# jeanfeydy/geomloss

Measured on AMD Instinct MI355X. Metric: softmin pairs/s, N=M=1e6 3D fp32 (Sinkhorn wall-clock: `sinkhorn_wallclock`; roofline: `roofline`), higher is better.
Workload: dtype f32

## Files before the change

### geomloss_amd/csrc/glhip_api.hip

```cpp
#include "glhip_autosort.h"
#include "glhip_launch.h"

namespace glhip {
thread_local char g_err[512] = "";
}

#define GL_NBP(DD) XdShape<DD>::NBP
static const int kXdNBP[] = {GL_NBP(4), GL_NBP(5), GL_NBP(6), GL_NBP(7), GL_NBP(8), GL_NBP(9), GL_NBP(10), GL_NBP(11), GL_NBP(12), GL_NBP(13), GL_NBP(14), GL_NBP(15), GL_NBP(16)};
#undef GL_NBP
static_assert(sizeof kXdNBP / sizeof kXdNBP[0] == kXdMaxD - 3, "one entry per dimension of the xd kernels");

extern "C" {

int glhip_version(void) { return GLHIP_VERSION; }

size_t glhip_workspace_bytes(int B, int N, int M, int D, int n_ranges) {
    const int nr = X32Layout<XL_BF16X3>::NR, nbp = (D > 3 && D <= kXdMaxD) ? kXdNBP[D - 4] : 0;
    size_t bytes = forward_workspace_bytes(B, N, M, D, n_ranges, nr, nbp);
    if (bytes > 0 && autosort_applies(B, N, M, D, n_ranges, 0)) {
        const size_t sorted = autosort_bytes(N, M, D) + forward_workspace_bytes(1, N, M, D, (N + kSortSlab - 1) / kSortSlab, nr, nbp);
        bytes = bytes > sorted ? bytes : sorted;
    }
    return bytes;
}
// ... 12 lines not shown
        sc.l2.groups = static_cast<const GroupBox*>(a.groups);
        sc.l2.home = a.home;
        sc.l2.t2 = a.t2;
        sc.l2.centre_x = x;
        sc.l2.n_groups = (M + 31) / 32;
        sc.l2.L2 = (float)(prune_L(M) * 1.4426950408889634);
    }
    const Ranges rg{a.ranges_i, a.slices_i, a.red};
    return (in_dtype == GLHIP_F32) ? softmin_fwd_typed<float>(fn, a.xs, a.ys, h, a.out, 1, N, M, D, eps, p, rg, a.C, sc, inner, st, step)
                                   : softmin_fwd_typed<bf16_t>(fn, a.xs, a.ys, h, a.out, 1, N, M, D, eps, p, rg, a.C, sc, inner, st, step);
}

int glhip_softmin_fwd_family(int B, long N, long M, int D, int p, int dtype, int flags, int n_ranges) {
    if (B < 0 || N < 0 || M < 0 || N > 0x7fffffffL || M > 0x7fffffffL || D < 1 || n_ranges < 0 || (p != 1 && p != 2) ||
        (dtype != GLHIP_F32 && dtype != GLHIP_BF16))
        return GLHIP_EINVAL;
    if (softmin_sorts(B, (int)N, (int)M, D, p, n_ranges, flags))
        return softmin_fwd_family(1, N, M, D, p, flags | (p == 1 ? GLHIP_FLAG_MFMA_DIST : 0) | GLHIP_FLAG_NO_SORT, (int)((N + kSortSlab - 1) / kSortSlab));
    return softmin_fwd_family(B, N, M, D, p, flags, n_ranges);
}

int glhip_softmin_perm_applies(int B, long N, long M, int D, int p, int dtype, int flags, int n_ranges) {
    if (B < 0 || N < 0 || M < 0 || N > 0x7fffffffL || M > 0x7fffffffL || D < 1 || n_ranges < 0 || (p != 1 && p != 2) ||
        (dtype != GLHIP_F32 && dtype != GLHIP_BF16))
        return GLHIP_EINVAL;
    return p == 2 && softmin_sorts(B, (int)N, (int)M, D, p, n_ranges, flags) ? 1 : 0;
}

static int softmin_step(const char* fn, const void* x, const void* y, const float* logw, const float* pot, const float* prev, float* out, int B,
                        int N, int M, int D, float eps, float damping, int p, int in_dtype, const int32_t* ranges_i, const int32_t* slices_i,
                        const int32_t* redranges_j, int n_ranges, void* workspace, size_t workspace_bytes, int flags, void* stream,
                        int32_t* perm_x = nullptr, int32_t* perm_y = nullptr, int perm_flags = 0) {
    int rc = check_common(fn, x, y, logw, B, N, M, D, in_dtype, ranges_i, slices_i, redranges_j, n_ranges);
    if (rc) return rc;
    if (B == 0 || N == 0) return GLHIP_OK;
    if (!out) return fail(GLHIP_EINVAL, "%s: NULL out", fn);
    if (out == prev) return fail(GLHIP_EINVAL, "%s: out must not alias prev (updates are simultaneous)", fn);
    if (!(eps > 0.f)) return fail(GLHIP_EINVAL, "%s: eps must be > 0", fn);
    if (p != 1 && p != 2) return fail(GLHIP_EUNSUPPORTED, "%s: p must be 1 or 2 (got %d)", fn, p);
    hipStream_t st = static_cast<hipStream_t>(stream);
    StepArgs step{pot, prev, prev ? 0.5f * damping : damping, prev ? 0.5f : 0.f};
    if (softmin_sorts(B, N, M, D, p, n_ranges, flags)) {
        AutoSort a;
        const int C = (N + kSortSlab - 1) / kSortSlab;
        rc = autosort_prepare(a, x, y, N, M, D, in_dtype, workspace, workspace_bytes, glhip_workspace_bytes(1, N, M, D, C), st, p == 1, perm_x,
                              perm_y, perm_flags);
        if (rc) return rc;
        if (a.on) {
            gather_f32(logw, a.perm_y, a.col0, M, st, a.hint_y);
            if (pot) { gather_f32(pot, a.perm_y, a.col1, M, st, a.hint_y); step.pot = a.col1; }
            if (prev) { gather_f32(prev, a.perm_x, a.row0, N, st, a.hint_x); step.prev = a.row0; }
            if (p == 2)
                prune_ranges(a.xs, a.ys, a.col0, step.pot, 1.0f / eps, N, M, D, in_dtype, eps, a.ranges_i, a.slices_i, a.red, a.blocks, a.groups, a.home,
                             a.t2, a.mlb, a.t1, st);
            rc = sorted_inner(fn, a, x, a.col0, N, M, D, eps, p, in_dtype, flags, st, step);
            if (rc) return rc;
            scatter_f32(a.out, a.perm_x, out, N, st, 1, a.hint_x);
            return check_launch(fn);
        }
    }
    const Ranges rg{ranges_i, slices_i, redranges_j};
    const Scratch sc = make_scratch(workspace, workspace_bytes, flags, n_ranges, N);
    rc = (in_dtype == GLHIP_F32) ? softmin_fwd_typed<float>(fn, x, y, logw, out, B, N, M, D, eps, p, rg, n_ranges, sc, flags, st, step)
                                 : softmin_fwd_typed<bf16_t>(fn, x, y, logw, out, B, N, M, D, eps, p, rg, n_ranges, sc, flags, st, step);
    return rc ? rc : check_launch(fn);
}

int glhip_softmin_fwd(const void* x, const void* y, const float* h, float* out, int B, int N, int M, int D,
                      float eps, int p, int in_dtype, const int32_t* ranges_i, const int32_t* slices_i,
                      const int32_t* redranges_j, int n_ranges, void* workspace, size_t workspace_bytes, int flags,
                      void* stream) {
    return softmin_step("glhip_softmin_fwd", x, y, h, nullptr, nullptr, out, B, N, M, D, eps, 1.f, p, in_dtype, ranges_i, slices_i, redranges_j,
                        n_ranges, workspace, workspace_bytes, flags, stream);
}

int glhip_sinkhorn_step(const void* x, const void* y, const float* logw, const float* pot, const float* prev,
                        float* out, int B, int N, int M, int D, float eps, float damping, int p, int in_dtype,
                        const int32_t* ranges_i, const int32_t* slices_i, const int32_t* redranges_j, int n_ranges,
                        void* workspace, size_t workspace_bytes, int flags, void* stream) {
    return softmin_step("glhip_sinkhorn_step", x, y, logw, pot, prev, out, B, N, M, D, eps, damping, p, in_dtype, ranges_i, slices_i, redranges_j,
                        n_ranges, workspace, workspace_bytes, flags, stream);
}

int glhip_sinkhorn_step_perm(const void* x, const void* y, const float* logw, const float* pot, const float* prev,
                             float* out, int B, int N, int M, int D, float eps, float damping, int p, int in_dtype,
                             const int32_t* ranges_i, const int32_t* slices_i, const int32_t* redranges_j, int n_ranges,
                             void* workspace, size_t workspace_bytes, int flags, void* stream, int32_t* perm_x, int32_t* perm_y,
                             int perm_flags) {
    return softmin_step("glhip_sinkhorn_step_perm", x, y, logw, pot, prev, out, B, N, M, D, eps, damping, p, in_dtype, ranges_i, slices_i,
                        redranges_j, n_ranges, workspace, workspace_bytes, flags, stream, perm_x, perm_y, perm_flags);
}

int glhip_prune_inspect_slots(int M) { return M > 0 ? prune_plan(M).S : GLHIP_EINVAL; }

int glhip_prune_inspect(const void* x, const void* y, const float* logw, const float* pot, int N, int M, int D, float eps, int in_dtype,
                        int32_t* perm_x, int32_t* perm_y, double* mlb, double* t1, int32_t* home, int32_t* intervals, float* t2,
                        void* workspace, size_t workspace_bytes, void* stream) {
    const char* fn = "glhip_prune_inspect";
    int rc = check_common(fn, x, y, logw, 1, N, M, D, in_dtype, nullptr, nullptr, nullptr, 0);
    if (rc) return rc;
    if (!(eps > 0.f)) return fail(GLHIP_EINVAL, "%s: eps must be > 0", fn);
    if (!softmin_sorts(1, N, M, D, 2, 0, 0))
        return fail(GLHIP_EUNSUPPORTED, "%s: a p = 2 call of this shape is not pruned (N = %d, M = %d, D = %d)", fn, N, M, D);
    hipStream_t st = static_cast<hipStream_t>(stream);
    AutoSort a;
    const int C = (N + kSortSlab - 1) / kSortSlab;
    rc = autosort_prepare(a, x, y, N, M, D, in_dtype, workspace, workspace_bytes, glhip_workspace_bytes(1, N, M, D, C), st, false);
    if (rc) return rc;
    if (!a.on) return fail(GLHIP_EINVAL, "%s: needs a workspace of glhip_workspace_bytes(1, N, M, D, 0)", fn);
    gather_f32(logw, a.perm_y, a.col0, M, st);
    if (pot) gather_f32(pot, a.perm_y, a.col1, M, st);
    if (hipMemsetD32Async(reinterpret_cast<hipDeviceptr_t>(a.t2), (int)0xFF800000u, (size_t)((N + 31) / 32), st) != hipSuccess)
        return fail(GLHIP_ELAUNCH, "%s: memset failed: %s", fn, hipGetErrorString(hipGetLastError()));
    prune_ranges(a.xs, a.ys, a.col0, pot ? a.col1 : nullptr, 1.0f / eps, N, M, D, in_dtype, eps, a.ranges_i, a.slices_i, a.red, a.blocks, a.groups,
                 a.home, a.t2, a.mlb, a.t1, st);
    auto copy = [&](void* dst, const void* src, size_t bytes) {
        return !dst || hipMemcpyAsync(dst, src, bytes, hipMemcpyDeviceToDevice, st) == hipSuccess;
    };
    const bool ok = copy(perm_x, a.perm_x, (size_t)N * 4) && copy(perm_y, a.perm_y, (size_t)M * 4) && copy(mlb, a.mlb, (size_t)C * 8) &&
                    copy(t1, a.t1, (size_t)C * 8) && copy(home, a.home, (size_t)C * 4) &&
                    copy(intervals, a.red, (size_t)C * prune_plan(M).S * 8) && copy(t2, a.t2, (size_t)((N + 31) / 32) * 4);
    if (!ok) return fail(GLHIP_ELAUNCH, "%s: copy failed: %s", fn, hipGetErrorString(hipGetLastError()));
    return check_launch(fn);
}

int glhip_sinkhorn_iter4(const void* x, const void* y, const float* a_log, const float* b_log, const float* f_ba,
                         const float* g_ab, const float* f_aa, const float* g_bb, float* f_ba_out, float* g_ab_out,
                         float* f_aa_out, float* g_bb_out, int B, int N, int M, int D, float eps, float damping, int p,
                         int in_dtype, int first, void* workspace, size_t workspace_bytes, int flags, void* stream) {
    int rc = check_common("glhip_sinkhorn_iter4", x, y, b_log, B, N, M, D, in_dtype, nullptr, nullptr, nullptr, 0);
    if (rc) return rc;
    if ((p != 1 && p != 2) || D > kXdMaxD) return fail(GLHIP_EUNSUPPORTED, "glhip_sinkhorn_iter4: only p = 1, 2 and D <= 16 (got p = %d, D = %d)", p, D);
    if (flags & (GLHIP_FLAG_DIRECT | GLHIP_FLAG_NO_MFMA | GLHIP_FLAG_F32_MFMA | GLHIP_FLAG_XDL16))
        return fail(GLHIP_EUNSUPPORTED, "glhip_sinkhorn_iter4: runs on the default 32x32x16 kernel only (flags = %d)", flags);
    if (B == 0 || N == 0 || M == 0) return GLHIP_OK;
    if (!a_log || !f_ba_out || !g_ab_out) return fail(GLHIP_EINVAL, "glhip_sinkhorn_iter4: NULL a_log / f_ba_out / g_ab_out");
    if ((f_aa_out == nullptr) != (g_bb_out == nullptr)) return fail(GLHIP_EINVAL, "glhip_sinkhorn_iter4: f_aa_out and g_bb_out go together");
    if (first < 0 || first > 2) return fail(GLHIP_EINVAL, "glhip_sinkhorn_iter4: first must be 0, 1 or 2 (got %d)", first);
    if (first != 1 && (!f_ba || !g_ab || (f_aa_out && (!f_aa || !g_bb))))
        return fail(GLHIP_EINVAL, "glhip_sinkhorn_iter4: NULL potential (only allowed with first = 1)");
    if (first != 1 && (f_ba_out == f_ba || g_ab_out == g_ab || (f_aa_out && (f_aa_out == f_aa || g_bb_out == g_bb))))
        return fail(GLHIP_EINVAL, "glhip_sinkhorn_iter4: outputs must not alias inputs (updates are simultaneous)");
    if (!(eps > 0.f)) return fail(GLHIP_EINVAL, "glhip_sinkhorn_iter4: eps must be > 0");
    hipStream_t st = static_cast<hipStream_t>(stream);
    const Scratch sc = make_scratch(workspace, workspace_bytes, flags & ~GLHIP_FLAG_PREPACK, 0, N);
    rc = (in_dtype == GLHIP_F32)
             ? iter4_typed<float>(x, y, a_log, b_log, f_ba, g_ab, f_aa, g_bb, f_ba_out, g_ab_out, f_aa_out, g_bb_out, B, N, M, D, eps, damping, p, first, sc, st)
             : iter4_typed<bf16_t>(x, y, a_log, b_log, f_ba, g_ab, f_aa, g_bb, f_ba_out, g_ab_out, f_aa_out, g_bb_out, B, N, M, D, eps, damping, p, first, sc, st);
    return rc ? rc : check_launch("glhip_sinkhorn_iter4");
}

int glhip_sinkhorn_anneal(const void* x, const void* y, const float* a_log, const float* b_log, float* const* set0, float* const* set1,
                          int B, int N, int M, int D, const float* eps, const float* damping, int n_eps, int p, int in_dtype,
                          void* workspace, size_t workspace_bytes, int flags, float f16x2_min_eps, void* stream) {
    const char* fn = "glhip_sinkhorn_anneal";
    int rc = check_common(fn, x, y, b_log, B, N, M, D, in_dtype, nullptr, nullptr, nullptr, 0);
    if (rc) return rc;
    if ((p != 1 && p != 2) || D > kXdMaxD) return fail(GLHIP_EUNSUPPORTED, "%s: only p = 1, 2 and D <= 16 (got p = %d, D = %d)", fn, p, D);
    if (flags & (GLHIP_FLAG_DIRECT | GLHIP_FLAG_NO_MFMA | GLHIP_FLAG_F32_MFMA | GLHIP_FLAG_XDL16))
        return fail(GLHIP_EUNSUPPORTED, "%s: runs on the default 32x32x16 kernel only (flags = %d)", fn, flags);
    if (n_eps < 1 || !eps || !damping) return fail(GLHIP_EINVAL, "%s: needs n_eps >= 1 temperatures and dampings (n_eps = %d)", fn, n_eps);
    if (B == 0 || N == 0 || M == 0) return GLHIP_OK;
    if (!a_log || !set0 || !set1) return fail(GLHIP_EINVAL, "%s: NULL a_log / set0 / set1", fn);
    float* const* sets[2] = {set0, set1};
    const bool debias = set0[2] != nullptr;
    for (int s = 0; s < 2; ++s) {
        if (!sets[s][0] || !sets[s][1]) return fail(GLHIP_EINVAL, "%s: NULL f_ba / g_ab buffer in set%d", fn, s);
        if ((sets[s][2] != nullptr) != debias || (sets[s][3] != nullptr) != debias)
// ... 51 lines not shown
```

### geomloss_amd/csrc/glhip_autosort.h

```cpp
#pragma once

#include <hip/hip_runtime.h>

#include <cmath>
#include <cstddef>
#include <cstdint>

#include "glhip_error.h"
#include "glhip_split_policy.h"

namespace glhip {

constexpr int kSortSlab = 256;
constexpr int kSortColChunks = 8;
constexpr int kSortRowsPerVoxel = 256;

constexpr int kPruneColBlock = 256;
constexpr int kPruneRuns = 160;
constexpr int kBalanceBlock = 1024;
constexpr int kBalanceLeaf = 32;
constexpr int kPruneGrid = 64;
constexpr double kPruneMarginNats = 1.0;
constexpr int kPruneBuckets = 112;
constexpr double kPruneBucketNats = 0.25;
constexpr double kPruneMassShare = 0.5;
constexpr double kPruneBudget1 = 1.4901161193847656e-08 * (1.0 - 1.0 / 2.718281828459045 - kPruneMassShare);
constexpr double kPruneBudget2 = 1.4901161193847656e-08 * kPruneMassShare;

struct PrunePlan {
    int nT;
    int PB;
    int S;
};
inline PrunePlan prune_plan(int M) {
    PrunePlan p;
    p.nT = (M + kPruneColBlock - 1) / kPruneColBlock;
    p.PB = (p.nT + kPruneGrid - 1) / kPruneGrid;
    p.PB = p.PB > 64 ? p.PB : 64;
    p.S = kPruneRuns + (p.nT + p.PB - 1) / p.PB;
    return p;
}
constexpr double kPruneMinPairs = 1e11;
inline bool prune_applies(int N, int M) {
    const long C = (N + kSortSlab - 1) / kSortSlab;
    return (double)N * M >= kPruneMinPairs && C * (long)prune_plan(M).S * 2 < (1L << 31) - 1;
}

size_t compact_sort_scratch_bytes(int n);
int compact_sort(const void* z, int n, int D, int in_dtype, int rows_per_voxel, int32_t* perm, void* z_sorted, void* scratch,
                 size_t scratch_bytes, hipStream_t st, int sub = 1, bool hinted = false);
void gather_f32(const float* src, const int32_t* perm, float* dst, int n, hipStream_t st, bool hinted = false);
void scatter_f32(const float* src, const int32_t* perm, float* dst, int n, hipStream_t st, int width = 1, bool hinted = false);
void slab_ranges(int N, int M, int32_t* ranges_i, int32_t* slices_i, int32_t* red, hipStream_t st);
size_t prune_blocks_bytes(int M);
size_t prune_groups_bytes(int M);
void prune_ranges(const void* xs, const void* ys, const float* h, const float* pot, float pot_scale, int N, int M, int D, int in_dtype,
                  float eps, int32_t* ranges_i, int32_t* slices_i, int32_t* red, void* blocks, void* groups, int32_t* home, float* t2,
                  double* mlb, double* t1, hipStream_t st);
inline double prune_L(int M) { return std::log((double)M) + 26.0 * 0.6931471805599453 + kPruneMarginNats; }
inline int prune_sort_sub(int D) { return D >= 3 ? 2 : (D == 2 ? 3 : 8); }

inline bool autosort_applies(int B, int N, int M, int D, int n_ranges, int flags) {
    return B == 1 && n_ranges == 0 && D <= 3 && N >= 65536 && (double)N * M >= 5e8 &&
           !(flags & (2  | 1  | 512 ));
}

struct AutoSort {
    bool on = false;
    int C = 0;
    int32_t *perm_x = nullptr, *perm_y = nullptr, *ranges_i = nullptr, *slices_i = nullptr, *red = nullptr;
    bool hint_x = false, hint_y = false;
    void *xs = nullptr, *ys = nullptr;
    float *col0 = nullptr, *col1 = nullptr, *row0 = nullptr, *out = nullptr;
    float* out_rows = nullptr;
    void* blocks = nullptr;
    void* groups = nullptr;
    int32_t* home = nullptr;
    float* t2 = nullptr;
    double *mlb = nullptr, *t1 = nullptr;
    void* inner_ws = nullptr;
    size_t inner_bytes = 0;
};

inline size_t autosort_bytes(int N, int M, int D) {
    const int C = (N + kSortSlab - 1) / kSortSlab;
    const int L = N > M ? N : M;
    const size_t slots = (size_t)(kSortColChunks > prune_plan(M).S ? kSortColChunks : prune_plan(M).S);
    return align256((size_t)N * 4) + align256((size_t)M * 4) + align256((size_t)N * D * 4) + align256((size_t)M * D * 4) +
           2 * align256((size_t)M * 4) + 2 * align256((size_t)N * 4) + align256((size_t)N * D * 4) + align256((size_t)C * 8) +
           align256((size_t)C * 4) +
           align256((size_t)C * slots * 8) + align256(prune_blocks_bytes(M)) + align256(prune_groups_bytes(M)) +
           align256((size_t)C * 4) + compact_sort_scratch_bytes(L);
}

inline int autosort_prepare(AutoSort& a, const void* x, const void* y, int N, int M, int D, int in_dtype, void* workspace,
                            size_t workspace_bytes, size_t inner_min, hipStream_t st, bool slabs = true, int32_t* ext_x = nullptr,
                            int32_t* ext_y = nullptr, int perm_flags = 0) {
    const size_t need = autosort_bytes(N, M, D);
    if (!workspace || workspace_bytes < need + inner_min) return 0;
    char* w = static_cast<char*>(workspace);
    size_t off = 0;
    auto take = [&](size_t bytes) { char* p = w + off; off += align256(bytes); return p; };
    a.C = (N + kSortSlab - 1) / kSortSlab;
    a.perm_x = reinterpret_cast<int32_t*>(take((size_t)N * 4));
    a.perm_y = reinterpret_cast<int32_t*>(take((size_t)M * 4));
    a.xs = take((size_t)N * D * 4);
    a.ys = take((size_t)M * D * 4);
    a.col0 = reinterpret_cast<float*>(take((size_t)M * 4));
    a.col1 = reinterpret_cast<float*>(take((size_t)M * 4));
    a.row0 = reinterpret_cast<float*>(take((size_t)N * 4));
    a.out = reinterpret_cast<float*>(take((size_t)N * 4));
    a.out_rows = reinterpret_cast<float*>(take((size_t)N * D * 4));
    a.ranges_i = reinterpret_cast<int32_t*>(take((size_t)a.C * 8));
    a.slices_i = reinterpret_cast<int32_t*>(take((size_t)a.C * 4));
    const size_t slots = (size_t)(kSortColChunks > prune_plan(M).S ? kSortColChunks : prune_plan(M).S);
    a.red = reinterpret_cast<int32_t*>(take((size_t)a.C * slots * 8));
    a.blocks = take(prune_blocks_bytes(M));
    a.groups = take(prune_groups_bytes(M));
    a.home = reinterpret_cast<int32_t*>(take((size_t)a.C * 4));
    const int L = N > M ? N : M;
    const size_t sb = compact_sort_scratch_bytes(L);
    void* scratch = take(sb);
    if (!slabs && ext_x) { a.perm_x = ext_x; a.hint_x = (perm_flags & 1) != 0; }
    if (!slabs && ext_y) { a.perm_y = ext_y; a.hint_y = (perm_flags & 2) != 0; }
    int rc = compact_sort(x, N, D, in_dtype, kSortRowsPerVoxel, a.perm_x, a.xs, scratch, sb, st, slabs ? 1 : prune_sort_sub(D), a.hint_x);
    if (rc) return rc;
    rc = compact_sort(y, M, D, in_dtype, slabs ? 2 * kSortRowsPerVoxel : kSortRowsPerVoxel, a.perm_y, a.ys, scratch, sb, st,
                      slabs ? 1 : prune_sort_sub(D), a.hint_y);
    if (rc) return rc;
    if (slabs) slab_ranges(N, M, a.ranges_i, a.slices_i, a.red, st);
    a.mlb = reinterpret_cast<double*>(scratch);
    a.t1 = a.mlb + a.C;
    a.t2 = reinterpret_cast<float*>(a.t1 + a.C);
    a.inner_ws = w + off;
    a.inner_bytes = workspace_bytes - off;
    a.on = true;
    return 0;
}

template <class Inner>
int autosort_conv(const char* fn, const void* x, const void* y, const float* v, float* out, float* rows_out, int N, int M, int D,
                  int in_dtype, void* workspace, size_t workspace_bytes, int flags, hipStream_t st, bool* ran, Inner inner) {
    AutoSort a;
    *ran = false;
    const int C = (N + kSortSlab - 1) / kSortSlab;
    int rc = autosort_prepare(a, x, y, N, M, D, in_dtype, workspace, workspace_bytes, glhip_workspace_bytes(1, N, M, D, C), st);
    if (rc || !a.on) return rc;
    *ran = true;
    gather_f32(v, a.perm_y, a.col0, M, st);
    rc = inner(a, flags | GLHIP_FLAG_MFMA_DIST | GLHIP_FLAG_NO_SORT);
    if (rc) return rc;
    scatter_f32(a.out, a.perm_x, out, N, st);
    if (rows_out) scatter_f32(a.out_rows, a.perm_x, rows_out, N, st, D);
    return check_launch(fn);
}

}
```

### geomloss_amd/csrc/glhip_prune.hip

```cpp
#include <climits>
#include <cmath>
#include <cstdint>

#include "glhip_autosort.h"
#include "glhip_common.h"
#include "glhip_prune_words.h"

using namespace glhip;

namespace {

struct ColBlock {
    float lo[3];
    float hmax;
    float hi[3];
    float lse;
};
constexpr float kPruneLseSlack = 9.5367431640625e-7f;
__device__ __forceinline__ float lse_up(float v) { return v + kPruneLseSlack * (__builtin_fabsf(v) + 8.f); }

static_assert(kHomeCols == kPruneColBlock && kPruneColBlock % 64 == 0 && sizeof(GroupBox) == 32, "block / group records");

template <typename T>
__global__ void __launch_bounds__(256) prune_blocks_kernel(const T* __restrict__ ys, const float* __restrict__ h, const float* __restrict__ pot,
                                                           float pot_scale, int M, int D, int nT, ColBlock* __restrict__ out,
                                                           GroupBox* __restrict__ groups) {
    const int lane = threadIdx.x & 63;
    const int t = blockIdx.x * 4 + (threadIdx.x >> 6);
    if (t >= nT) return;
    float blo[3] = {INFINITY, INFINITY, INFINITY}, bhi[3] = {-INFINITY, -INFINITY, -INFINITY};
    float bhm = -INFINITY;
    float gls[kPruneColBlock / 64];
    int bbad = 0;
    const int j0 = t * kPruneColBlock, j1 = min(M, j0 + kPruneColBlock);
#pragma unroll
    for (int k = 0; k < kPruneColBlock / 64; ++k) {
        float lo[3] = {INFINITY, INFINITY, INFINITY}, hi[3] = {-INFINITY, -INFINITY, -INFINITY};
        float hm = -INFINITY, hv = -INFINITY;
        int bad = 0;
        const int j = j0 + 64 * k + lane;
        if (j < j1) {
            for (int d = 0; d < D; ++d) {
                const float v = to_f32<T>(ys[(long)j * D + d]);
                bad |= !__builtin_isfinite(v);
                lo[d] = v;
                hi[d] = v;
            }
            hv = pot ? __builtin_fmaf(pot[j], pot_scale, h[j]) : h[j];
            bad |= __builtin_isnan(hv);
            hm = fmaxf(hm, hv);
        }
        for (int off = 16; off > 0; off >>= 1) {
            for (int d = 0; d < D; ++d) {
                lo[d] = fminf(lo[d], __shfl_xor(lo[d], off, 64));
                hi[d] = fmaxf(hi[d], __shfl_xor(hi[d], off, 64));
            }
            hm = fmaxf(hm, __shfl_xor(hm, off, 64));
            bad |= __shfl_xor(bad, off, 64);
        }
        float se = (__builtin_isfinite(hm) && hv > -INFINITY) ? expf(hv - hm) : 0.f;
        for (int off = 16; off > 0; off >>= 1) se += __shfl_xor(se, off, 64);
        const float gl = __builtin_isfinite(hm) ? lse_up(hm + logf(se)) : hm;
        gls[k] = gl;
        const int g0 = j0 + 64 * k + (lane & 32);
        if ((lane & 31) == 0 && g0 < j1) {
            GroupBox b;
            for (int d = 0; d < 3; ++d) {
                b.lohi[d][0] = d < D ? lo[d] : 0.f;
                b.lohi[d][1] = d < D ? hi[d] : 0.f;
            }
            b.lse = gl;
            b.special = bad;
// ... 34 lines not shown
        b.lse = bbad ? NAN : blse;
        out[t] = b;
    }
}

__device__ __forceinline__ void box_d2(const double (&rlo)[3], const double (&rhi)[3], const ColBlock& b, int D, double& dmin2, double& dmax2) {
    dmin2 = 0.0;
    dmax2 = 0.0;
    for (int d = 0; d < D; ++d) {
        const double blo = b.lo[d], bhi = b.hi[d];
        const double gap = fmax(fmax(blo - rhi[d], rlo[d] - bhi), 0.0);
        const double far = fmax(bhi - rlo[d], rhi[d] - blo);
        dmin2 = fma(gap, gap, dmin2);
        dmax2 = fma(far, far, dmax2);
    }
}

template <bool MAX>
__device__ __forceinline__ int block_scan256(int v, int* buf) {
    const int t = threadIdx.x;
    buf[t] = v;
    __syncthreads();
    for (int off = 1; off < 256; off <<= 1) {
        const int o = t >= off ? buf[t - off] : (MAX ? INT_MIN : 0);
        __syncthreads();
        v = MAX ? max(v, o) : v + o;
        buf[t] = v;
        __syncthreads();
    }
    return v;
}

__device__ __forceinline__ int prune_bucket(double key, double lo) {
    const double d = (key - lo) * (1.0 / kPruneBucketNats);
    if (d < 0.0) return -1;
    return d < (double)kPruneBuckets ? (int)d : kPruneBuckets;
}
__device__ __forceinline__ int prune_first_kept(const double* hist, double under, double budget) {
    double s = under;
    int b = 0;
    for (; b < kPruneBuckets; ++b) {
        if (s + hist[b] > budget) break;
        s += hist[b];
    }
    return b;
}

constexpr int kPruneMaskWords = 1024;
constexpr int kPruneGaps = 2048;
template <typename T>
__global__ void __launch_bounds__(256) prune_slabs_kernel(const T* __restrict__ xs, int N, int M, int D, const ColBlock* __restrict__ blocks,
                                                          int nT, int PB, int S, double inv2eps, double L, int32_t* __restrict__ ranges_i,
                                                          int32_t* __restrict__ slices_i, int32_t* __restrict__ red, int32_t* __restrict__ home,
                                                          double* __restrict__ mlb_out, double* __restrict__ t1_out) {
    __shared__ int buf[256];
    __shared__ double hist[kPruneBuckets + 1];
    __shared__ int first_kept;
    __shared__ unsigned long long mask[kPruneMaskWords];
    __shared__ int32_t gaps[kPruneGaps];
    __shared__ float wlo[4][3], whi[4][3];
    __shared__ double wm[4];
    __shared__ int wb[4];
    const int k = blockIdx.x, tid = threadIdx.x, lane = tid & 63, wave = tid >> 6;
    const int r0 = k * kSortSlab, r1 = min(N, r0 + kSortSlab);
    if (tid == 0) {
        ranges_i[2 * k] = r0;
        ranges_i[2 * k + 1] = r1;
        slices_i[k] = (k + 1) * S;
    }
    float lo[3] = {INFINITY, INFINITY, INFINITY}, hi[3] = {-INFINITY, -INFINITY, -INFINITY};
    int bad = 0;
    if (r0 + tid < r1) {
        for (int d = 0; d < D; ++d) {
            const float v = to_f32<T>(xs[(long)(r0 + tid) * D + d]);
            bad |= !__builtin_isfinite(v);
            lo[d] = v;
            hi[d] = v;
        }
    }
    for (int d = 0; d < D; ++d) {
        for (int off = 32; off > 0; off >>= 1) {
            lo[d] = fminf(lo[d], __shfl_xor(lo[d], off, 64));
            hi[d] = fmaxf(hi[d], __shfl_xor(hi[d], off, 64));
        }
        if (lane == 0) { wlo[wave][d] = lo[d]; whi[wave][d] = hi[d]; }
    }
    bad = __syncthreads_or(bad);
    double rlo[3] = {0.0, 0.0, 0.0}, rhi[3] = {0.0, 0.0, 0.0};
    for (int d = 0; d < D; ++d) {
        rlo[d] = fminf(fminf(wlo[0][d], wlo[1][d]), fminf(wlo[2][d], wlo[3][d]));
        rhi[d] = fmaxf(fmaxf(whi[0][d], whi[1][d]), fmaxf(whi[2][d], whi[3][d]));
    }
    double mlb = -INFINITY;
    int best = -1;
    if (!bad) {
        for (int t = tid; t < nT; t += 256) {
            const ColBlock b = blocks[t];
            if (__builtin_isnan(b.lse)) continue;
            double dmin2, dmax2;
            box_d2(rlo, rhi, b, D, dmin2, dmax2);
            const double v = (double)b.hmax - dmax2 * inv2eps;
            if (v > mlb) { mlb = v; best = t; }
        }
        auto take = [&](double v, int t) {
            if (t >= 0 && (v > mlb || (v == mlb && (best < 0 || t < best)))) { mlb = v; best = t; }
        };
        for (int off = 32; off > 0; off >>= 1) {
            const double v = __shfl_xor(mlb, off, 64);
            const int t = __shfl_xor(best, off, 64);
            take(v, t);
        }
        if (lane == 0) { wm[wave] = mlb; wb[wave] = best; }
        __syncthreads();
        mlb = -INFINITY;
        best = -1;
        for (int w = 0; w < 4; ++w) take(wm[w], wb[w]);
    }
    const bool keep_all = bad || !__builtin_isfinite(mlb);
    const double lo_key = mlb - L;
    auto block_key = [&](const ColBlock& b) {
        double dmin2, dmax2;
        box_d2(rlo, rhi, b, D, dmin2, dmax2);
        return (double)b.lse - dmin2 * inv2eps;
    };
    for (int q = tid; q <= kPruneBuckets; q += 256) hist[q] = 0.0;
    __syncthreads();
    if (!keep_all) {
        for (int t = tid; t < nT; t += 256) {
            const ColBlock b = blocks[t];
            if (__builtin_isnan(b.lse)) continue;
            const double key = block_key(b);
            const int q = prune_bucket(key, lo_key);
            if (q >= kPruneBuckets) continue;
            const double mass = exp(key - mlb);
            if (mass > 0.0) atomicAdd(&hist[q < 0 ? kPruneBuckets : q], mass);
        }
    }
    __syncthreads();
    if (tid == 0) {
        first_kept = keep_all ? 0 : prune_first_kept(hist, hist[kPruneBuckets], kPruneBudget1);
        mlb_out[k] = mlb;
        t1_out[k] = keep_all ? -INFINITY : lo_key + first_kept * kPruneBucketNats;
    }
    __syncthreads();
    const int fk = first_kept;
    auto kept = [&](int t) {
        if (keep_all) return true;
        const ColBlock b = blocks[t];
        if (__builtin_isnan(b.lse)) return true;
        return prune_bucket(block_key(b), lo_key) >= fk;
    };
    const int nW = (nT + 63) >> 6;
    const bool masked = nW <= kPruneMaskWords;
    {
        int all = 1;
        if (masked) {
            for (int w = wave; w < nW; w += 4) {
                const int t = 64 * w + lane;
                const unsigned long long m = __ballot(t < nT && kept(t));
                if (lane == 0) mask[w] = m;
                all &= m == (nT - 64 * w >= 64 ? ~0ull : (1ull << (nT - 64 * w)) - 1ull);
            }
        } else if (!keep_all) {
            for (int t = tid; t < nT && all; t += 256) all = kept(t) ? 1 : 0;
        }
        all = __syncthreads_and(all);
        if (tid == 0) home[k] = (keep_all || all) ? -1 : best;
    }
    auto kept_at = [&](int t) { return masked ? ((mask[t >> 6] >> (t & 63)) & 1ull) != 0 : kept(t); };
    int32_t* slots = red + 2 * (long)k * S;
    auto walk = [&](int g, bool emit) {
        int carry = -1, runs = 0, pieces = 0;
        for (int c0 = 0; c0 < nT; c0 += 256) {
            const int t = c0 + tid;
            const bool kp = t < nT && kept_at(t);
            block_scan256<true>(kp ? t : -1, buf);
            const int prev = max(carry, tid > 0 ? buf[tid - 1] : -1);
            const int last = buf[255];
            const bool run = kp && (prev < 0 || t - prev - 1 >= g);
            const bool start = run || (kp && t % PB == 0);
            runs += __syncthreads_count(run);
            carry = max(carry, last);
            if (emit) {
                const int idx = pieces + block_scan256<false>(start ? 1 : 0, buf) - 1;
                if (start && idx < S) {
                    slots[2 * idx] = t * kPruneColBlock;
                    if (idx > 0) slots[2 * idx - 1] = min(M, (run ? prev + 1 : t) * kPruneColBlock);
                }
                pieces += __syncthreads_count(start);
            }
        }
        if (emit) {
            const int n = min(pieces, S);
            if (tid == 0 && n > 0) slots[2 * n - 1] = min(M, (carry + 1) * kPruneColBlock);
            for (int q = n + tid; q < S; q += 256) {
                slots[2 * q] = 0;
                slots[2 * q + 1] = 0;
            }
        }
        return runs;
    };
    const int wpt = (nW + 255) / 256, w0 = min(nW, tid * wpt), w1 = min(nW, w0 + wpt);
    int runs1 = 0;
    if (masked) {
        auto emit_words = [&](int gw, int nstart) {
            const int base = block_scan256<false>(nstart, buf) - nstart;
            const int n = min(buf[255], S);
            prune_emit_words(mask, w0, w1, base, PB, S, kPruneColBlock, M, slots, gw);
            if (tid == 0 && n > 0) prune_emit_last(mask, nW, n, kPruneColBlock, M, slots);
            for (int q = n + tid; q < S; q += 256) {
                slots[2 * q] = 0;
                slots[2 * q + 1] = 0;
            }
        };
        int nrun, nstart;
        prune_count_words(mask, w0, w1, PB, nrun, nstart);
        const int run0 = block_scan256<false>(nrun, buf) - nrun;
        runs1 = buf[255];
        __syncthreads();
        if (runs1 <= kPruneRuns) {
            emit_words(1, nstart);
            return;
        }
        if (runs1 - 1 <= kPruneGaps) {
            const int n_gaps = runs1 - 1;
            prune_gap_lengths(mask, w0, w1, run0, kPruneGaps, gaps);
            __syncthreads();
            int lo_g = 0, hi_g = nT;
            while (hi_g - lo_g > 1) {
                const int mid = lo_g + (hi_g - lo_g) / 2;
                int c = 0;
                for (int q0 = 0; q0 < n_gaps; q0 += 256) c += __syncthreads_count(q0 + tid < n_gaps && gaps[q0 + tid] >= mid);
                if (1 + c > kPruneRuns) lo_g = mid; else hi_g = mid;
            }
            prune_count_words(mask, w0, w1, PB, nrun, nstart, hi_g);
            emit_words(hi_g, nstart);
            return;
        }
    }
    int g = 1;
    if ((masked ? runs1 : walk(1, false)) > kPruneRuns) {
        int lo_g = 1, hi_g = nT;
        while (hi_g - lo_g > 1) {
            const int mid = lo_g + (hi_g - lo_g) / 2;
            if (walk(mid, false) > kPruneRuns) lo_g = mid; else hi_g = mid;
        }
        g = hi_g;
    }
    walk(g, true);
}

static_assert(kPruneRuns + kPruneGrid <= 256 && kSortSlab == 256, "one thread per interval slot / per row");
template <typename T>
__global__ void __launch_bounds__(256) prune_tiles_kernel(const T* __restrict__ xs, const T* __restrict__ ys, const float* __restrict__ h,
                                                          const float* __restrict__ pot, float pot_scale, int N, int M, int D,
                                                          const GroupBox* __restrict__ groups, const int32_t* __restrict__ red, int S,
                                                          const int32_t* __restrict__ home, double inv2eps, double L, float* __restrict__ t2) {
    constexpr int kTiles = kSortSlab / 32;
    __shared__ int buf[256];
    __shared__ int first_group[256];
    __shared__ double hy[kPruneColBlock][3], hh[kPruneColBlock];
    __shared__ float tlo[kTiles][3], thi[kTiles][3];
    __shared__ double ms[kTiles];
    __shared__ double hist[kTiles][kPruneBuckets + 1];
    const int k = blockIdx.x, tid = threadIdx.x, w = tid >> 5;
    const int hb = home[k];
    if (hb < 0) return;
    const int r0 = k * kSortSlab, r1 = min(N, r0 + kSortSlab);
    {
        const int j = hb * kPruneColBlock + tid;
        const bool real = j < M;
        for (int d = 0; d < 3; ++d) hy[tid][d] = (real && d < D) ? (double)to_f32<T>(ys[(long)j * D + d]) : 0.0;
        hh[tid] = real ? (double)(pot ? __builtin_fmaf(pot[j], pot_scale, h[j]) : h[j]) : -INFINITY;
    }
    for (int q = tid; q < kTiles * (kPruneBuckets + 1); q += 256) (&hist[0][0])[q] = 0.0;
    const bool row = r0 + tid < r1;
    float x[3] = {0.f, 0.f, 0.f};
    if (row)
        for (int d = 0; d < D; ++d) x[d] = to_f32<T>(xs[(long)(r0 + tid) * D + d]);
    for (int d = 0; d < 3; ++d) {
        float lo = row ? x[d] : INFINITY, hi = row ? x[d] : -INFINITY;
        for (int off = 16; off > 0; off >>= 1) {
            lo = fminf(lo, __shfl_xor(lo, off, 64));
            hi = fmaxf(hi, __shfl_xor(hi, off, 64));
        }
        if ((tid & 31) == 0) { tlo[w][d] = lo; thi[w][d] = hi; }
    }
    __syncthreads();
    {
        double seed = -INFINITY;
        const double xd[3] = {(double)x[0], (double)x[1], (double)x[2]};
        for (int j = 0; j < kPruneColBlock; ++j) {
            double d2 = 0.0;
            for (int d = 0; d < 3; ++d) {
                const double t = xd[d] - hy[j][d];
                d2 = fma(t, t, d2);
            }
            seed = fmax(seed, hh[j] - d2 * inv2eps);
        }
        int ok = !row || __builtin_isfinite(seed);
        double v = row ? seed : INFINITY;
        for (int off = 16; off > 0; off >>= 1) {
            v = fmin(v, __shfl_xor(v, off, 64));
            ok &= __shfl_xor(ok, off, 64);
        }
        if ((tid & 31) == 0) ms[w] = (ok && r0 + 32 * w < r1) ? v : NAN;
    }
    const int32_t* slots = red + 2 * (long)k * S;
    int j0 = 0, ng = 0;
    if (tid < S) {
        j0 = slots[2 * tid];
        ng = (max(slots[2 * tid + 1], j0) - j0 + 31) >> 5;
    }
    const int incl = block_scan256<false>(ng, buf);
    first_group[tid] = incl - ng;
    const int total = buf[255];
    __syncthreads();
    const int c = tid & (kTiles - 1), sub = tid / kTiles;
    const double m = ms[c], lo_key = m - L;
    double tl[3], th[3];
    for (int d = 0; d < 3; ++d) {
        tl[d] = (double)tlo[c][d];
        th[d] = (double)thi[c][d];
    }
    double under = 0.0;
    for (int f0 = 0; f0 < total; f0 += 256) {
        const int f = f0 + tid;
        int g = 0;
        if (f < total) {
            int q = 0;
            for (int step = 128; step > 0; step >>= 1)
                if (q + step < 256 && first_group[q + step] <= f) q += step;
            g = (slots[2 * q] >> 5) + (f - first_group[q]);
        }
        __syncthreads();
        buf[tid] = g;
        __syncthreads();
        if (!(m == m)) continue;
        const int cnt = min(256, total - f0);
        for (int s = sub; s < cnt; s += 2 * (256 / kTiles)) {
            const int s1 = s + 256 / kTiles;
            const GroupBox b0 = groups[buf[s]], b1 = groups[buf[min(s1, cnt - 1)]];
#pragma unroll
            for (int u = 0; u < 2; ++u) {
                const GroupBox& b = u ? b1 : b0;
                if ((u && s1 >= cnt) || b.special) continue;
                double dmin2 = 0.0;
                for (int d = 0; d < 3; ++d) {
                    const double gap = fmax(fmax((double)b.lohi[d][0] - th[d], tl[d] - (double)b.lohi[d][1]), 0.0);
                    dmin2 = fma(gap, gap, dmin2);
                }
                const double key = (double)b.lse - dmin2 * inv2eps;
                const int bk = prune_bucket(key, lo_key);
                if (bk >= kPruneBuckets) continue;
                const double mass = exp(key - m);
                if (bk < 0) under += mass;
                else if (mass > 0.0) atomicAdd(&hist[c][bk], mass);
            }
        }
    }
    if (under > 0.0) atomicAdd(&hist[c][kPruneBuckets], under);
    __syncthreads();
    if (tid < kTiles && r0 + 32 * tid < r1) {
        const double m = ms[tid];
        float out = -INFINITY;
        if (m == m) {
            const int fk = prune_first_kept(hist[tid], hist[tid][kPruneBuckets], kPruneBudget2);
            const double v = (m - L + fk * kPruneBucketNats) * 1.4426950408889634;
            out = (float)v;
            if ((double)out > v) out = nextafterf(out, -INFINITY);
        }
        t2[(r0 >> 5) + tid] = out;
    }
}

template <typename T>
void prune_ranges_typed(const void* xs_, const void* ys_, const float* h, const float* pot, float pot_scale, int N, int M, int D, float eps,
                        int32_t* ranges_i, int32_t* slices_i, int32_t* red, void* blocks_, void* groups_, int32_t* home, float* t2,
                        double* mlb, double* t1, hipStream_t st) {
    const T *xs = static_cast<const T*>(xs_), *ys = static_cast<const T*>(ys_);
    const PrunePlan pp = prune_plan(M);
    const int C = (N + kSortSlab - 1) / kSortSlab;
    ColBlock* blocks = static_cast<ColBlock*>(blocks_);
    GroupBox* groups = static_cast<GroupBox*>(groups_);
    const double inv2eps = 0.5 / (double)eps;
    const double L = prune_L(M);
    hipLaunchKernelGGL(prune_blocks_kernel<T>, dim3((pp.nT + 3) / 4), dim3(256), 0, st, ys, h, pot, pot_scale, M, D, pp.nT, blocks, groups);
    hipLaunchKernelGGL(prune_slabs_kernel<T>, dim3(C), dim3(256), 0, st, xs, N, M, D, blocks, pp.nT, pp.PB, pp.S, inv2eps, L, ranges_i, slices_i,
                       red, home, mlb, t1);
    hipLaunchKernelGGL(prune_tiles_kernel<T>, dim3(C), dim3(256), 0, st, xs, ys, h, pot, pot_scale, N, M, D, groups, red, pp.S, home, inv2eps, L,
                       t2);
}

}

namespace glhip {

size_t prune_blocks_bytes(int M) { return (size_t)prune_plan(M).nT * sizeof(ColBlock); }
size_t prune_groups_bytes(int M) { return (size_t)((M + 31) / 32) * sizeof(GroupBox); }

void prune_ranges(const void* xs, const void* ys, const float* h, const float* pot, float pot_scale, int N, int M, int D, int in_dtype,
                  float eps, int32_t* ranges_i, int32_t* slices_i, int32_t* red, void* blocks, void* groups, int32_t* home, float* t2,
                  double* mlb, double* t1, hipStream_t st) {
    if (in_dtype == GLHIP_F32) prune_ranges_typed<float>(xs, ys, h, pot, pot_scale, N, M, D, eps, ranges_i, slices_i, red, blocks, groups, home, t2, mlb, t1, st);
    else prune_ranges_typed<bf16_t>(xs, ys, h, pot, pot_scale, N, M, D, eps, ranges_i, slices_i, red, blocks, groups, home, t2, mlb, t1, st);
}

}
```

### include/glhip.h

```cpp
#ifndef GLHIP_H
#define GLHIP_H

#include <stddef.h>
#include <stdint.h>

#ifdef __cplusplus
extern "C" {
#endif

#define GLHIP_VERSION 135

#define GLHIP_F32 0
#define GLHIP_BF16 1

#define GLHIP_GAUSSIAN 0
#define GLHIP_LAPLACIAN 1
#define GLHIP_ENERGY 2

#define GLHIP_FLAG_DIRECT 1
#define GLHIP_FLAG_NO_MFMA 2
#define GLHIP_FLAG_NO_SPLIT 4
#define GLHIP_FLAG_F32_MFMA 8
#define GLHIP_FLAG_XDL16 16
#define GLHIP_FLAG_GRAD_FAMILY GLHIP_FLAG_XDL16
#define GLHIP_FLAG_PREPACK 32
#define GLHIP_FLAG_MFMA_DIST 64
#define GLHIP_FLAG_SMALL_ROW_BLOCKS 128

#define GLHIP_FLAG_F16X2 256

#define GLHIP_FLAG_XK_GRAD 1024

#define GLHIP_FLAG_XK_DIST 2048

#define GLHIP_FLAG_XK_DIST_GRAD 4096

#define GLHIP_DIST_GRAD_SOFTMIN_P1 0
#define GLHIP_DIST_GRAD_LAPLACIAN 1
#define GLHIP_DIST_GRAD_ENERGY 2

#define GLHIP_FLAG_NO_SORT 512


#define GLHIP_OK 0
#define GLHIP_EINVAL (-1)
#define GLHIP_EUNSUPPORTED (-2)
#define GLHIP_ELAUNCH (-3)

#define GLHIP_FAMILY_VALU 0
#define GLHIP_FAMILY_X32 1
#define GLHIP_FAMILY_XD 2
#define GLHIP_FAMILY_XK 3
#define GLHIP_FAMILY_DIST 4
#define GLHIP_FAMILY_GENERIC 5

int glhip_version(void);
const char* glhip_last_error(void);

size_t glhip_workspace_bytes(int B, int N, int M, int D, int n_ranges);

int glhip_softmin_fwd_family(int B, long N, long M, int D, int p, int dtype, int flags, int n_ranges);
int glhip_kernel_conv_fwd_family(int kind, int B, long N, long M, int D, int dtype, int flags, int n_ranges);

// ... 162 lines not shown
```

Before: 65190 billion.

## Tighten pruning budgets with lower bounds on the log-sum-exp mass

Computes a lower bound on each slab's and tile's log-sum-exp, using worst-case (farthest) box distances over all column blocks and over a short list of reference groups. The pruning error budgets are scaled up by exp(lower bound − max), so more column blocks and tiles can be discarded. This cuts the work done by the softmin inner loop. In exchange it adds a sum pass, reference-list bookkeeping in the slab kernel and a per-row exp loop over up to 128 reference groups in the tile kernel. The workspace layout also gains a refs array, which is not visibly added to the workspace size calculation.

```diff
diff --git a/geomloss_amd/csrc/glhip_api.hip b/geomloss_amd/csrc/glhip_api.hip
--- a/geomloss_amd/csrc/glhip_api.hip
+++ b/geomloss_amd/csrc/glhip_api.hip
@@ -88,7 +88,7 @@
             if (prev) { gather_f32(prev, a.perm_x, a.row0, N, st, a.hint_x); step.prev = a.row0; }
             if (p == 2)
                 prune_ranges(a.xs, a.ys, a.col0, step.pot, 1.0f / eps, N, M, D, in_dtype, eps, a.ranges_i, a.slices_i, a.red, a.blocks, a.groups, a.home,
-                             a.t2, a.mlb, a.t1, st);
+                             a.t2, a.mlb, a.t1, a.refs, st);
             rc = sorted_inner(fn, a, x, a.col0, N, M, D, eps, p, in_dtype, flags, st, step);
             if (rc) return rc;
             scatter_f32(a.out, a.perm_x, out, N, st, 1, a.hint_x);
@@ -149,7 +149,7 @@
     if (hipMemsetD32Async(reinterpret_cast<hipDeviceptr_t>(a.t2), (int)0xFF800000u, (size_t)((N + 31) / 32), st) != hipSuccess)
         return fail(GLHIP_ELAUNCH, "%s: memset failed: %s", fn, hipGetErrorString(hipGetLastError()));
     prune_ranges(a.xs, a.ys, a.col0, pot ? a.col1 : nullptr, 1.0f / eps, N, M, D, in_dtype, eps, a.ranges_i, a.slices_i, a.red, a.blocks, a.groups,
-                 a.home, a.t2, a.mlb, a.t1, st);
+                 a.home, a.t2, a.mlb, a.t1, a.refs, st);
     auto copy = [&](void* dst, const void* src, size_t bytes) {
         return !dst || hipMemcpyAsync(dst, src, bytes, hipMemcpyDeviceToDevice, st) == hipSuccess;
     };
diff --git a/geomloss_amd/csrc/glhip_autosort.h b/geomloss_amd/csrc/glhip_autosort.h
--- a/geomloss_amd/csrc/glhip_autosort.h
+++ b/geomloss_amd/csrc/glhip_autosort.h
@@ -26,6 +26,12 @@
 constexpr double kPruneMassShare = 0.5;
 constexpr double kPruneBudget1 = 1.4901161193847656e-08 * (1.0 - 1.0 / 2.718281828459045 - kPruneMassShare);
 constexpr double kPruneBudget2 = 1.4901161193847656e-08 * kPruneMassShare;
+constexpr int kPruneRefBlocks = 16;
+constexpr double kPruneRefTop = 5.625;
+constexpr int kPruneRefCellsPerNat = 16;
+constexpr int kPruneRefCells = 512;
+constexpr double kPruneSumSlack = 1e-9;
+constexpr double kPruneLsSlack = 1e-4;
 
 struct PrunePlan {
     int nT;
@@ -56,7 +62,7 @@
 size_t prune_groups_bytes(int M);
 void prune_ranges(const void* xs, const void* ys, const float* h, const float* pot, float pot_scale, int N, int M, int D, int in_dtype,
                   float eps, int32_t* ranges_i, int32_t* slices_i, int32_t* red, void* blocks, void* groups, int32_t* home, float* t2,
-                  double* mlb, double* t1, hipStream_t st);
+                  double* mlb, double* t1, int32_t* refs, hipStream_t st);
 inline double prune_L(int M) { return std::log((double)M) + 26.0 * 0.6931471805599453 + kPruneMarginNats; }
 inline int prune_sort_sub(int D) { return D >= 3 ? 2 : (D == 2 ? 3 : 8); }
 
@@ -78,6 +84,7 @@
     int32_t* home = nullptr;
     float* t2 = nullptr;
     double *mlb = nullptr, *t1 = nullptr;
+    int32_t* refs = nullptr;
     void* inner_ws = nullptr;
     size_t inner_bytes = 0;
 };
@@ -129,9 +136,11 @@
                       slabs ? 1 : prune_sort_sub(D), a.hint_y);
     if (rc) return rc;
     if (slabs) slab_ranges(N, M, a.ranges_i, a.slices_i, a.red, st);
+    static_assert(kPruneRefBlocks <= 256, "the reference lists stay under 4 bytes per row");
     a.mlb = reinterpret_cast<double*>(scratch);
     a.t1 = a.mlb + a.C;
     a.t2 = reinterpret_cast<float*>(a.t1 + a.C);
+    a.refs = reinterpret_cast<int32_t*>(a.t2 + (N + 31) / 32);
     a.inner_ws = w + off;
     a.inner_bytes = workspace_bytes - off;
     a.on = true;
diff --git a/geomloss_amd/csrc/glhip_prune.hip b/geomloss_amd/csrc/glhip_prune.hip
--- a/geomloss_amd/csrc/glhip_prune.hip
+++ b/geomloss_amd/csrc/glhip_prune.hip
@@ -18,6 +18,14 @@
 };
 constexpr float kPruneLseSlack = 9.5367431640625e-7f;
 __device__ __forceinline__ float lse_up(float v) { return v + kPruneLseSlack * (__builtin_fabsf(v) + 8.f); }
+__device__ __forceinline__ double lse_dn(float v, double times) {
+    return (double)v - times * (double)kPruneLseSlack * ((double)__builtin_fabsf(v) + 8.0);
+}
+__device__ __forceinline__ int prune_ref_cell(double score, double mlb) {
+    const double q = (mlb + kPruneRefTop - score) * (double)kPruneRefCellsPerNat;
+    if (!(q < (double)kPruneRefCells)) return kPruneRefCells;
+    return q > 0.0 ? (int)q : 0;
+}
 
 static_assert(kHomeCols == kPruneColBlock && kPruneColBlock % 64 == 0 && sizeof(GroupBox) == 32, "block / group records");
 
@@ -158,10 +166,12 @@
 __global__ void __launch_bounds__(256) prune_slabs_kernel(const T* __restrict__ xs, int N, int M, int D, const ColBlock* __restrict__ blocks,
                                                           int nT, int PB, int S, double inv2eps, double L, int32_t* __restrict__ ranges_i,
                                                           int32_t* __restrict__ slices_i, int32_t* __restrict__ red, int32_t* __restrict__ home,
-                                                          double* __restrict__ mlb_out, double* __restrict__ t1_out) {
+                                                          double* __restrict__ mlb_out, double* __restrict__ t1_out, int32_t* __restrict__ refs_out) {
     __shared__ int buf[256];
     __shared__ double hist[kPruneBuckets + 1];
     __shared__ int first_kept;
+    __shared__ int cells[kPruneRefCells];
+    __shared__ int ref_cells, ref_n, ref_l[kPruneRefBlocks];
     __shared__ unsigned long long mask[kPruneMaskWords];
     __shared__ int32_t gaps[kPruneGaps];
     __shared__ float wlo[4][3], whi[4][3];
@@ -230,26 +240,49 @@
         return (double)b.lse - dmin2 * inv2eps;
     };
     for (int q = tid; q <= kPruneBuckets; q += 256) hist[q] = 0.0;
-    __syncthreads();
+    for (int q = tid; q < kPruneRefCells; q += 256) cells[q] = 0;
+    if (tid == 0) ref_n = 0;
+    __syncthreads();
+    double ssum = 0.0;
     if (!keep_all) {
         for (int t = tid; t < nT; t += 256) {
             const ColBlock b = blocks[t];
             if (__builtin_isnan(b.lse)) continue;
-            const double key = block_key(b);
+            double dmin2, dmax2;
+            box_d2(rlo, rhi, b, D, dmin2, dmax2);
+            const double score = lse_dn(b.lse, 4.0) - dmax2 * inv2eps;
+            if (score - mlb > -40.0) ssum += exp(score - mlb);
+            const int cell = prune_ref_cell(score, mlb);
+            if (cell < kPruneRefCells) atomicAdd(&cells[cell], 1);
+            const double key = (double)b.lse - dmin2 * inv2eps;
             const int q = prune_bucket(key, lo_key);
             if (q >= kPruneBuckets) continue;
             const double mass = exp(key - mlb);
             if (mass > 0.0) atomicAdd(&hist[q < 0 ? kPruneBuckets : q], mass);
         }
     }
+    for (int off = 32; off > 0; off >>= 1) ssum += __shfl_xor(ssum, off, 64);
+    __syncthreads();
+    if (lane == 0) wm[wave] = ssum;
     __syncthreads();
     if (tid == 0) {
-        first_kept = keep_all ? 0 : prune_first_kept(hist, hist[kPruneBuckets], kPruneBudget1);
+        const double sum = (wm[0] + wm[1]) + (wm[2] + wm[3]);
+        double slb = mlb;
+        if (!keep_all && sum > 0.0 && __builtin_isfinite(sum)) slb = fmax(mlb, mlb + log(sum) - kPruneSumSlack);
+        first_kept = keep_all ? 0 : prune_first_kept(hist, hist[kPruneBuckets], kPruneBudget1 * exp(slb - mlb));
         mlb_out[k] = mlb;
         t1_out[k] = keep_all ? -INFINITY : lo_key + first_kept * kPruneBucketNats;
-    }
-    __syncthreads();
-    const int fk = first_kept;
+        int nc = 0;
+        for (int n = 0; nc < kPruneRefCells && n + cells[nc] <= kPruneRefBlocks - 1; ++nc) n += cells[nc];
+        ref_cells = nc;
+    }
+    __syncthreads();
+    const int fk = first_kept, rc = ref_cells;
+    auto ref_take = [&](int t, const ColBlock& b, double dmax2) {
+        if (t != best && prune_ref_cell(lse_dn(b.lse, 4.0) - dmax2 * inv2eps, mlb) >= rc) return;
+        const int i = atomicAdd(&ref_n, 1);
+        if (i < kPruneRefBlocks) ref_l[i] = t;
+    };
     auto kept = [&](int t) {
         if (keep_all) return true;
         const ColBlock b = blocks[t];
@@ -263,15 +296,42 @@
         if (masked) {
             for (int w = wave; w < nW; w += 4) {
                 const int t = 64 * w + lane;
-                const unsigned long long m = __ballot(t < nT && kept(t));
+                bool kp = t < nT;
+                if (kp && !keep_all) {
+                    const ColBlock b = blocks[t];
+                    if (!__builtin_isnan(b.lse)) {
+                        double dmin2, dmax2;
+                        box_d2(rlo, rhi, b, D, dmin2, dmax2);
+                        kp = prune_bucket((double)b.lse - dmin2 * inv2eps, lo_key) >= fk;
+                        ref_take(t, b, dmax2);
+                    }
+                }
+                const unsigned long long m = __ballot(kp);
                 if (lane == 0) mask[w] = m;
                 all &= m == (nT - 64 * w >= 64 ? ~0ull : (1ull << (nT - 64 * w)) - 1ull);
             }
         } else if (!keep_all) {
             for (int t = tid; t < nT && all; t += 256) all = kept(t) ? 1 : 0;
+            for (int t = tid; t < nT; t += 256) {
+                const ColBlock b = blocks[t];
+                if (__builtin_isnan(b.lse)) continue;
+                double dmin2, dmax2;
+                box_d2(rlo, rhi, b, D, dmin2, dmax2);
+                ref_take(t, b, dmax2);
+            }
         }
         all = __syncthreads_and(all);
         if (tid == 0) home[k] = (keep_all || all) ? -1 : best;
+        if (tid < kPruneRefBlocks) {
+            const int n = min(ref_n, kPruneRefBlocks);
+            int rank = tid, v = -1;
+            if (tid < n) {
+                v = ref_l[tid];
+                rank = 0;
+                for (int j = 0; j < n; ++j) rank += ref_l[j] < v;
+            }
+            refs_out[(long)k * kPruneRefBlocks + rank] = v;
+        }
     }
     auto kept_at = [&](int t) { return masked ? ((mask[t >> 6] >> (t & 63)) & 1ull) != 0 : kept(t); };
     int32_t* slots = red + 2 * (long)k * S;
@@ -356,13 +416,21 @@
     walk(g, true);
 }
 
+struct RefGroup {
+    float lo[3], hi[3];
+    double dn;
+};
+constexpr int kRefGroups = kPruneRefBlocks * (kPruneColBlock / 32);
 static_assert(kPruneRuns + kPruneGrid <= 256 && kSortSlab == 256, "one thread per interval slot / per row");
 template <typename T>
 __global__ void __launch_bounds__(256) prune_tiles_kernel(const T* __restrict__ xs, const T* __restrict__ ys, const float* __restrict__ h,
                                                           const float* __restrict__ pot, float pot_scale, int N, int M, int D,
                                                           const GroupBox* __restrict__ groups, const int32_t* __restrict__ red, int S,
-                                                          const int32_t* __restrict__ home, double inv2eps, double L, float* __restrict__ t2) {
+                                                          const int32_t* __restrict__ home, const int32_t* __restrict__ refs, double inv2eps,
+                                                          double L, float* __restrict__ t2) {
     constexpr int kTiles = kSortSlab / 32;
+    __shared__ RefGroup rg[kRefGroups];
+    __shared__ double lsw[kTiles];
     __shared__ int buf[256];
     __shared__ int first_group[256];
     __shared__ double hy[kPruneColBlock][3], hh[kPruneColBlock];
@@ -380,6 +448,25 @@
         hh[tid] = real ? (double)(pot ? __builtin_fmaf(pot[j], pot_scale, h[j]) : h[j]) : -INFINITY;
     }
     for (int q = tid; q < kTiles * (kPruneBuckets + 1); q += 256) (&hist[0][0])[q] = 0.0;
+    const int n_ref = __syncthreads_count(tid < kPruneRefBlocks && refs[(long)k * kPruneRefBlocks + tid] >= 0);
+    for (int q = tid; q < n_ref * (kPruneColBlock / 32); q += 256) {
+        const int t = refs[(long)k * kPruneRefBlocks + q / (kPruneColBlock / 32)];
+        const long g = (long)t * (kPruneColBlock / 32) + q % (kPruneColBlock / 32);
+        RefGroup r;
+        for (int d = 0; d < 3; ++d) r.lo[d] = r.hi[d] = 0.f;
+        r.dn = -INFINITY;
+        if (t >= 0 && t < (M + kPruneColBlock - 1) / kPruneColBlock && g < (M + 31) / 32) {
+            const GroupBox b = groups[g];
+            if (!b.special && !__builtin_isnan(b.lse)) {
+                for (int d = 0; d < 3; ++d) {
+                    r.lo[d] = b.lohi[d][0];
+                    r.hi[d] = b.lohi[d][1];
+                }
+                r.dn = lse_dn(b.lse, 2.0);
+            }
+        }
+        rg[q] = r;
+    }
     const bool row = r0 + tid < r1;
     float x[3] = {0.f, 0.f, 0.f};
     if (row)
@@ -406,11 +493,36 @@
         }
         int ok = !row || __builtin_isfinite(seed);
         double v = row ? seed : INFINITY;
+        double ls = INFINITY;
+        if (row && __builtin_isfinite(seed)) {
+            double mref = seed;
+            float acc = 0.f;
+            for (int q = 0; q < n_ref * (kPruneColBlock / 32); ++q) {
+                const RefGroup& r = rg[q];
+                double d2 = 0.0;
+                for (int d = 0; d < 3; ++d) {
+                    const double far = fmax(fabs(xd[d] - (double)r.lo[d]), fabs((double)r.hi[d] - xd[d]));
+                    d2 = fma(far, far, d2);
+                }
+                double arg = r.dn - d2 * inv2eps - mref;
+                if (arg > 60.0) {
+                    acc *= __expf((float)-arg);
+                    mref += arg;
+                    arg = 0.0;
+                }
+                acc += __expf((float)arg);
+            }
+            ls = fmax(seed, mref + (double)logf(acc) - kPruneLsSlack);
+        }
         for (int off = 16; off > 0; off >>= 1) {
             v = fmin(v, __shfl_xor(v, off, 64));
+            ls = fmin(ls, __shfl_xor(ls, off, 64));
             ok &= __shfl_xor(ok, off, 64);
         }
-        if ((tid & 31) == 0) ms[w] = (ok && r0 + 32 * w < r1) ? v : NAN;
+        if ((tid & 31) == 0) {
+            ms[w] = (ok && r0 + 32 * w < r1) ? v : NAN;
+            lsw[w] = (__builtin_isfinite(ls) && ls > v) ? ls : v;
+        }
     }
     const int32_t* slots = red + 2 * (long)k * S;
     int j0 = 0, ng = 0;
@@ -471,7 +583,7 @@
         const double m = ms[tid];
         float out = -INFINITY;
         if (m == m) {
-            const int fk = prune_first_kept(hist[tid], hist[tid][kPruneBuckets], kPruneBudget2);
+            const int fk = prune_first_kept(hist[tid], hist[tid][kPruneBuckets], kPruneBudget2 * exp(lsw[tid] - m));
             const double v = (m - L + fk * kPruneBucketNats) * 1.4426950408889634;
             out = (float)v;
             if ((double)out > v) out = nextafterf(out, -INFINITY);
@@ -483,7 +595,7 @@
 template <typename T>
 void prune_ranges_typed(const void* xs_, const void* ys_, const float* h, const float* pot, float pot_scale, int N, int M, int D, float eps,
                         int32_t* ranges_i, int32_t* slices_i, int32_t* red, void* blocks_, void* groups_, int32_t* home, float* t2,
-                        double* mlb, double* t1, hipStream_t st) {
+                        double* mlb, double* t1, int32_t* refs, hipStream_t st) {
     const T *xs = static_cast<const T*>(xs_), *ys = static_cast<const T*>(ys_);
     const PrunePlan pp = prune_plan(M);
     const int C = (N + kSortSlab - 1) / kSortSlab;
@@ -493,8 +605,8 @@
     const double L = prune_L(M);
     hipLaunchKernelGGL(prune_blocks_kernel<T>, dim3((pp.nT + 3) / 4), dim3(256), 0, st, ys, h, pot, pot_scale, M, D, pp.nT, blocks, groups);
     hipLaunchKernelGGL(prune_slabs_kernel<T>, dim3(C), dim3(256), 0, st, xs, N, M, D, blocks, pp.nT, pp.PB, pp.S, inv2eps, L, ranges_i, slices_i,
-                       red, home, mlb, t1);
-    hipLaunchKernelGGL(prune_tiles_kernel<T>, dim3(C), dim3(256), 0, st, xs, ys, h, pot, pot_scale, N, M, D, groups, red, pp.S, home, inv2eps, L,
+                       red, home, mlb, t1, refs);
+    hipLaunchKernelGGL(prune_tiles_kernel<T>, dim3(C), dim3(256), 0, st, xs, ys, h, pot, pot_scale, N, M, D, groups, red, pp.S, home, refs, inv2eps, L,
                        t2);
 }
 
@@ -507,9 +619,9 @@
 
 void prune_ranges(const void* xs, const void* ys, const float* h, const float* pot, float pot_scale, int N, int M, int D, int in_dtype,
                   float eps, int32_t* ranges_i, int32_t* slices_i, int32_t* red, void* blocks, void* groups, int32_t* home, float* t2,
-                  double* mlb, double* t1, hipStream_t st) {
-    if (in_dtype == GLHIP_F32) prune_ranges_typed<float>(xs, ys, h, pot, pot_scale, N, M, D, eps, ranges_i, slices_i, red, blocks, groups, home, t2, mlb, t1, st);
-    else prune_ranges_typed<bf16_t>(xs, ys, h, pot, pot_scale, N, M, D, eps, ranges_i, slices_i, red, blocks, groups, home, t2, mlb, t1, st);
-}
-
-}
+                  double* mlb, double* t1, int32_t* refs, hipStream_t st) {
+    if (in_dtype == GLHIP_F32) prune_ranges_typed<float>(xs, ys, h, pot, pot_scale, N, M, D, eps, ranges_i, slices_i, red, blocks, groups, home, t2, mlb, t1, refs, st);
+    else prune_ranges_typed<bf16_t>(xs, ys, h, pot, pot_scale, N, M, D, eps, ranges_i, slices_i, red, blocks, groups, home, t2, mlb, t1, refs, st);
+}
+
+}
diff --git a/include/glhip.h b/include/glhip.h
--- a/include/glhip.h
+++ b/include/glhip.h
@@ -8,7 +8,7 @@
 extern "C" {
 #endif
 
-#define GLHIP_VERSION 135
+#define GLHIP_VERSION 136
 
 #define GLHIP_F32 0
 #define GLHIP_BF16 1
```

New measurement: 69360 billion, median of 6. 1.06x the previous value.
